# tennisonliu/bayesian-neural-network

Measured on AMD Instinct MI355X. Metric: MC-forward-samples/sec + KL-elements/sec, 784-1200-1200-10 BNN, higher is better.
Workload: dtype bf16

## Files before the change

bayesian-neural-network_amd/csrc/bbb_linear.hip:

```cpp
#include "bnn_device.h"
#include "bnn_fin.h"
#include "bbb_sample_body.h"
#include "bbb_block_gemm.h"
#include "../../include/bnn_hip.h"
#include <string.h>

namespace bnn {

struct BbbK {
  const void* x;
  long x_sstride;
  const float* w_mu;
  const float* w_rho;
  const float* w_sigma;
  const float* b_mu;
  const float* b_rho;
  const float* eps_w;
  const float* eps_b;
  float* eps_w_dump;
  float* eps_b_dump;
  void* y;
  float4* ws;
  int S, B, K, N;
  __bf16* y16;
// ... 801 lines not shown
}

template <int MATH, int R, bool ALIGNED>
__global__ __launch_bounds__(768) void bbb_input_grad_kernel(const BbbK p) {
  bbb_fwd_body<MATH, BNN_F32, R, ALIGNED, false, true>(p, nullptr);
}

template <int NW, bool SIG, int EPS>
__device__ __forceinline__ void bbb_gemm_body(const BbbK& p, float4 (*xt)[8 * 64], float (*bias_s)[16]) {
  const int lane = threadIdx.x & 63, wave = __builtin_amdgcn_readfirstlane(threadIdx.x >> 6);
  const int r = lane & 15, q = lane >> 4;
  const int K = p.K, N = p.N, B = p.B;
  const int tbs = (N + 16 * NW - 1) / (16 * NW), mbs = (B + 127) >> 7;
  const int KS = p.ksl;
  int tb, unit, ks;
  if (!xcd2d_work_item(p.xc, tb, unit, ks)) return;
  const int s = unit / mbs, mb = unit - s * mbs;
  const int item = tb * (p.S * mbs) + unit;
  const int tile = tb * NW + wave;
  const int n = tile * 16 + r;
  const bool n_ok = n < N;
  const int nc = min(n, N - 1);
  const int m0 = mb * 128;
  const int ksteps = (K + 31) >> 5;
  const int spb = (ksteps + KS - 1) / KS, t_lo = ks * spb, t_hi = min(ksteps, t_lo + spb);
  const uint32_t gs = global_sample(p, s);
  const bool do_stats = p.want_stats && mb == 0;
  const bool do_ls = do_stats && s == 0;
  const bool do_dump = mb == 0;
  const int gpr = (K + 3) >> 2;
  const uint32_t wid = p.layer_id * 4u;
  const __bf16* xs = reinterpret_cast<const __bf16*>(p.x) + (size_t)(s / p.xg) * (size_t)p.x_sstride;
  const int T = (N + 15) >> 4;

  if (do_stats && item == 0 && ks == 0 && threadIdx.x == 0) p.ws[0] = make_float4(__int_as_float(T * KS), 0.f, 0.f, 0.f);

  size_t xrow[8 / NW];
#pragma unroll
  for (int i = 0; i < 8 / NW; ++i) xrow[i] = (size_t)min(m0 + (wave + i * NW) * 16 + r, B - 1) * K;
  const uint32_t voff_w = ((uint32_t)nc * (uint32_t)K + (uint32_t)(q * 8)) * 4u, voff_w_max = ((uint32_t)nc * (uint32_t)K + (uint32_t)(K - 8)) * 4u;
  uint32_t voff_x[8 / NW], voff_x_max[8 / NW];
#pragma unroll
  for (int i = 0; i < 8 / NW; ++i) {
    voff_x[i] = ((uint32_t)xrow[i] + (uint32_t)(q * 8)) * 2u;
    voff_x_max[i] = ((uint32_t)xrow[i] + (uint32_t)(K - 8)) * 2u;
  }
  auto stage_dma = [&](int t, int buf) __attribute__((always_inline)) {
#pragma unroll
    for (int i = 0; i < 8 / NW; ++i) {
      const uint32_t vo = min(voff_x[i] + (uint32_t)t * 64u, voff_x_max[i]);
      const uint32_t m0v = (uint32_t)(size_t)(__attribute__((address_space(3))) void*)&xt[buf][(wave + i * NW) * 64];
      asm volatile("s_mov_b32 m0, %2\n\ts_nop 0\n\tglobal_load_lds_dwordx4 %0, %1" ::"v"(vo), "s"(xs), "s"(m0v) : "memory", "m0");
    }
  };

  struct PSet { float4 m_lo, m_hi, g_lo, g_hi; };
  auto load_params = [&](int t, PSet& P) __attribute__((always_inline)) {
    const uint32_t woff = min(voff_w + (uint32_t)t * 128u, voff_w_max);
    const float4* pm = reinterpret_cast<const float4*>(reinterpret_cast<const char*>(p.w_mu) + woff);
    const float4* pg = reinterpret_cast<const float4*>(reinterpret_cast<const char*>(SIG ? p.w_sigma : p.w_rho) + woff);
    P.m_lo = pm[0]; P.m_hi = pm[1]; P.g_lo = pg[0]; P.g_hi = pg[1];
  };

  float bmu_pre = 0.f, brho_pre = 0.f, beps_pre = 0.f;
  if (q == 0 && n_ok && ks == 0) {
    bmu_pre = p.b_mu[n];
    brho_pre = p.b_rho[n];
    beps_pre = bias_eps(p, n, s, gs, do_dump);
  }

  PSet PA, PB;
  PA.m_lo = PA.m_hi = PA.g_lo = PA.g_hi = PB.m_lo = PB.m_hi = PB.g_lo = PB.g_hi = make_float4(0.f, 0.f, 0.f, 0.f);
  if (t_lo < t_hi) {
    load_params(t_lo, PA);
    stage_dma(t_lo, t_lo & 1);
  }
  asm volatile("s_waitcnt vmcnt(0)" ::: "memory");
  __syncthreads();

  f32x4 acc[8];
#pragma unroll
  for (int m = 0; m < 8; ++m) acc[m] = f32x4{0.f, 0.f, 0.f, 0.f};
  float s_e2 = 0.f, s_a = 0.f, s_ls = 0.f;

  auto step = [&](int t, const PSet& P, PSet& Pn, auto more_) __attribute__((always_inline)) {
    constexpr bool more = decltype(more_)::value;
    const int k = t * 32 + q * 8;
    const bool lane_ok = n_ok && k < K;
#ifdef BNN_TUNE
    if (more) {
      if (!(p.tune & 8)) stage_dma(t + 1, (t + 1) & 1);
      if (!(p.tune & 4)) load_params(t + 1, Pn);
    }
#else
    if (more) {
      stage_dma(t + 1, (t + 1) & 1);
      load_params(t + 1, Pn);
    }
#endif
    const float mu[8] = {P.m_lo.x, P.m_lo.y, P.m_lo.z, P.m_lo.w, P.m_hi.x, P.m_hi.y, P.m_hi.z, P.m_hi.w};
    float sg[8] = {P.g_lo.x, P.g_lo.y, P.g_lo.z, P.g_lo.w, P.g_hi.x, P.g_hi.y, P.g_hi.z, P.g_hi.w};
    float e[8], w[8];
    if (EPS == BNN_EPS_PHILOX) {
      const uint32_t g = (uint32_t)n * (uint32_t)gpr + (uint32_t)(k >> 2);
      philox_normal8(g, gs, wid, p.k0, p.k1, e);
    } else if (EPS == BNN_EPS_MEMORY) {
      load8<true>(p.eps_w + ((size_t)s * N + n) * K + k, lane_ok ? 8 : 0, e);
    } else {
#pragma unroll
      for (int j = 0; j < 8; ++j) e[j] = 0.f;
    }
    if (p.eps_w_dump && do_dump) store8<true>(p.eps_w_dump + ((size_t)s * N + n) * K + k, lane_ok ? 8 : 0, e);
    float e2 = 0.f, a = 0.f, ls = 0.f;
#pragma unroll
    for (int j = 0; j < 8; ++j) {
      if (!SIG) sg[j] = softplus(sg[j]);
      w[j] = __builtin_fmaf(sg[j], e[j], mu[j]);
      e2 = __builtin_fmaf(e[j], e[j], e2);
    }
    if (do_stats) {
      if (p.prior_kind == BNN_PRIOR_GAUSS) {
#pragma unroll
        for (int j = 0; j < 8; ++j) a = __builtin_fmaf(w[j], w[j], a);
      } else {
#pragma unroll
        for (int j = 0; j < 8; ++j) a = add_log(a, mix_p(p, w[j]));
      }
      if (do_ls) {
#pragma unroll
        for (int j = 0; j < 8; ++j) ls = add_log(ls, sg[j]);
      }
      s_e2 += lane_ok ? e2 : 0.f;
      s_a += lane_ok ? a : 0.f;
      s_ls += lane_ok ? ls : 0.f;
    }
    bf16x8 wa;
#pragma unroll
    for (int j = 0; j < 8; ++j) wa[j] = lane_ok ? (__bf16)w[j] : (__bf16)0.f;
    const uint32_t xa = (uint32_t)(size_t)(__attribute__((address_space(3))) void*)&xt[t & 1][q * 16 + r];
#ifdef BNN_TUNE
    const bool tune_nolds = (p.tune & 16) != 0, tune_nomfma = (p.tune & 32) != 0;
#else
    constexpr bool tune_nolds = false, tune_nomfma = false;
#endif
#pragma unroll
    for (int h = 0; h < 2; ++h) {
      f32x4 x0, x1, x2, x3;
      if (tune_nolds) {
        x0 = x1 = x2 = x3 = f32x4{mu[0], mu[1], mu[2], mu[3]};
      } else {
        if (h == 0)
          asm volatile("ds_read_b128 %0, %4\n\tds_read_b128 %1, %4 offset:1024\n\tds_read_b128 %2, %4 offset:2048\n\tds_read_b128 %3, %4 offset:3072"
                       : "=&v"(x0), "=&v"(x1), "=&v"(x2), "=&v"(x3) : "v"(xa));
        else
          asm volatile("ds_read_b128 %0, %4 offset:4096\n\tds_read_b128 %1, %4 offset:5120\n\tds_read_b128 %2, %4 offset:6144\n\tds_read_b128 %3, %4 offset:7168"
                       : "=&v"(x0), "=&v"(x1), "=&v"(x2), "=&v"(x3) : "v"(xa));
        asm volatile("s_waitcnt lgkmcnt(0)" : "+v"(x0), "+v"(x1), "+v"(x2), "+v"(x3));
      }
      if (!tune_nomfma) {
        acc[h * 4 + 0] = __builtin_amdgcn_mfma_f32_16x16x32_bf16(wa, __builtin_bit_cast(bf16x8, x0), acc[h * 4 + 0], 0, 0, 0);
        acc[h * 4 + 1] = __builtin_amdgcn_mfma_f32_16x16x32_bf16(wa, __builtin_bit_cast(bf16x8, x1), acc[h * 4 + 1], 0, 0, 0);
        acc[h * 4 + 2] = __builtin_amdgcn_mfma_f32_16x16x32_bf16(wa, __builtin_bit_cast(bf16x8, x2), acc[h * 4 + 2], 0, 0, 0);
        acc[h * 4 + 3] = __builtin_amdgcn_mfma_f32_16x16x32_bf16(wa, __builtin_bit_cast(bf16x8, x3), acc[h * 4 + 3], 0, 0, 0);
      } else {
        asm volatile("" :: "v"(x0), "v"(x1), "v"(x2), "v"(x3));
      }
    }
#ifdef BNN_TUNE
    if (!(p.tune & 2)) asm volatile("s_waitcnt vmcnt(0)" ::: "memory");
    if (!(p.tune & 1)) __syncthreads();
#else
    asm volatile("s_waitcnt vmcnt(0)" ::: "memory");
    __syncthreads();
#endif
  };
  {
    int t = t_lo;
#pragma nounroll
    for (; t + 2 < t_hi; t += 2) {
      step(t, PA, PB, std::true_type{});
      step(t + 1, PB, PA, std::true_type{});
    }
    if (t + 1 < t_hi) {
      step(t, PA, PB, std::true_type{});
      step(t + 1, PB, PA, std::false_type{});
    } else if (t < t_hi) {
      step(t, PA, PB, std::false_type{});
    }
  }

  if (q == 0) {
    float b = 0.f;
    if (n_ok && ks == 0) b = sample_bias(p, bmu_pre, brho_pre, beps_pre, do_stats, do_ls, s_e2, s_a, s_ls);
    bias_s[wave][r] = b;
  }
  if (do_stats) {
    const float a = wave_sum(s_e2), b = wave_sum(s_a), cc = wave_sum(s_ls);
    if (lane == 0 && tile < T) p.ws[1 + ((size_t)s * T + tile) * KS + ks] = make_float4(a, b, cc, 0.f);
  }
  __syncthreads();
  const int nb = tile * 16 + q * 4;
  const bool vec_ok = (N & 3) == 0;
  float bq[4];
#pragma unroll
  for (int i = 0; i < 4; ++i) bq[i] = bias_s[wave][q * 4 + i];
  if (KS > 1) {
    __shared__ uint32_t last_s;
    float4* const unit_part = p.ks_part + (size_t)item * KS * (NW * 8 * 64);
    float4* const mine = unit_part + ((size_t)ks * NW + wave) * (8 * 64) + lane;
#pragma unroll
    for (int m = 0; m < 8; ++m) {
      f32x4 v = acc[m];
#pragma unroll
      for (int i = 0; i < 4; ++i) v[i] += bq[i];
      acc[m] = v;
      asm volatile("global_store_dwordx4 %0, %1, off sc1" ::"v"(mine + m * 64), "v"(v) : "memory");
    }
    asm volatile("s_waitcnt vmcnt(0)" ::: "memory");
    __syncthreads();
    if (threadIdx.x == 0) {
      const uint32_t tk = __hip_atomic_fetch_add(p.ks_ticket + item, 1u, __ATOMIC_RELAXED, __HIP_MEMORY_SCOPE_AGENT);
      last_s = (tk == (uint32_t)KS - 1u) ? 1u : 0u;
    }
    __syncthreads();
    if (last_s == 0u) return;
    if (threadIdx.x == 0) __hip_atomic_store(p.ks_ticket + item, 0u, __ATOMIC_RELAXED, __HIP_MEMORY_SCOPE_AGENT);
    f32x4 sum[8];
#pragma unroll
    for (int m = 0; m < 8; ++m) sum[m] = f32x4{0.f, 0.f, 0.f, 0.f};
#pragma nounroll
    for (int j = 0; j < KS; ++j) {
      f32x4 part[8];
      if (j != ks) {
        const float4* src = unit_part + ((size_t)j * NW + wave) * (8 * 64) + lane;
#pragma unroll
        for (int m = 0; m < 8; ++m)
          asm volatile("global_load_dwordx4 %0, %1, off sc1" : "=v"(part[m]) : "v"(src + m * 64) : "memory");
        asm volatile("s_waitcnt vmcnt(0)" ::: "memory");
      } else {
#pragma unroll
        for (int m = 0; m < 8; ++m) part[m] = acc[m];
      }
#pragma unroll
      for (int m = 0; m < 8; ++m) sum[m] += part[m];
    }
#pragma unroll
    for (int m = 0; m < 8; ++m) acc[m] = sum[m];
#pragma unroll
    for (int i = 0; i < 4; ++i) bq[i] = 0.f;
  }
  if (nb < N) {
#pragma unroll
    for (int m = 0; m < 8; ++m) {
      const int brow = m0 + m * 16 + r;
      if (brow < B) {
        f32x4 v = acc[m];
#pragma unroll
        for (int i = 0; i < 4; ++i) {
          float o = v[i] + bq[i];
          if (p.relu) o = fmaxf(o, 0.f);
          v[i] = o;
        }
        const size_t yoff = ((size_t)s * B + brow) * N + nb;
        if (p.y_bf16) {
          __bf16* yp = reinterpret_cast<__bf16*>(p.y) + yoff;
          if (vec_ok) {
            bf16x4 o;
#pragma unroll
            for (int i = 0; i < 4; ++i) o[i] = (__bf16)v[i];
            *reinterpret_cast<bf16x4*>(yp) = o;
          } else {
#pragma unroll
            for (int i = 0; i < 4; ++i)
              if (nb + i < N) yp[i] = (__bf16)v[i];
          }
        } else {
          float* yp = reinterpret_cast<float*>(p.y) + yoff;
          if (vec_ok) {
            *reinterpret_cast<float4*>(yp) = make_float4(v[0], v[1], v[2], v[3]);
          } else {
#pragma unroll
            for (int i = 0; i < 4; ++i)
              if (nb + i < N) yp[i] = v[i];
          }
        }
      }
    }
  }
}

template <int NW, bool SIG, int EPS>
__global__ __launch_bounds__(NW * 64, 4) void bbb_fwd_gemm_kernel(const BbbK p) {
  __shared__ __attribute__((aligned(16))) float4 xt[2][8 * 64];
  __shared__ float bias_s[NW][16];
  bbb_gemm_body<NW, SIG, EPS>(p, xt, bias_s);
}

template <int NF, int SB, int EPS, int NB = 2, bool X3 = false, int LAY = 0>
__global__ __launch_bounds__(NF * SB * 64, 4) void bbb_fwd_gemm2_kernel(const BbbK p) {
  constexpr int NW = NF * SB;
  constexpr bool XTL = (LAY & 1) != 0, YTL = (LAY & 2) != 0, WTL = (LAY & 4) != 0;
  static_assert(!X3 || LAY == 0, "piece order: bf16 form only");
  static_assert(NB == 2, "two staging buffers");
  constexpr int WPW = 4 / SB;
  constexpr int XPW = 8 / NF;
  constexpr int XT = X3 ? 1024 : 512;
  static_assert(SB == 1 || SB == 2 || SB == 4, "pairs per block");
  static_assert(NF == 2 || NF == 4 || NF == 8, "feature waves per block");
  constexpr int BUF = NF * 256 + SB * XT;
  auto p_idx = [](int buf) { return X3 ? 0 : buf * BUF; };
  auto x_idx = [](int buf) { return X3 ? NF * 256 + buf * (SB * XT) : buf * BUF + NF * 256; };
  __shared__ __attribute__((aligned(16))) float4 sm_all[X3 ? NF * 256 + 2 * SB * XT : NB * BUF + NW * 4];
  float (*bias_s)[16] = reinterpret_cast<float (*)[16]>(sm_all + (X3 ? 0 : NB * BUF));
  const int lane = threadIdx.x & 63, wave = __builtin_amdgcn_readfirstlane(threadIdx.x >> 6);
  const int fw = wave % NF, sb = wave / NF;
  const int r = lane & 15, q = lane >> 4;
  const int K = p.K, N = p.N, B = p.B;
  const int mbs = (B + 127) >> 7;
  const int U = p.S * mbs;
  int tb, ub, in_;
  if (!xcd2d_work_item(p.xc, tb, ub, in_)) return;
  const int unit_raw = ub * SB + sb;
  const bool active = unit_raw < U;
  const int unit = active ? unit_raw : U - 1;
  const int s = unit / mbs, mb = unit - s * mbs;
  const int tile = tb * NF + fw;
  const int n = tile * 16 + r;
  const bool n_ok = n < N;
  const int nc = min(n, N - 1);
  const int m0 = mb * 128;
  const int ksteps = (K + 31) >> 5;
  const uint32_t gs = global_sample(p, s);
  const bool do_stats = p.want_stats && mb == 0 && active;
  const bool do_ls = do_stats && s == 0;
  const bool do_dump = mb == 0 && active;
  const int gpr = (K + 3) >> 2;
  const uint32_t wid = p.layer_id * 4u;
  const __bf16* xs = reinterpret_cast<const __bf16*>(p.x) + (size_t)(s / p.xg) * (size_t)p.x_sstride;
  const __bf16* xs_lo = X3 ? reinterpret_cast<const __bf16*>(p.x_lo) + (size_t)(s / p.xg) * (size_t)p.x_sstride : nullptr;
  const int T = (N + 15) >> 4;

  if (do_stats && tb == 0 && unit == 0 && fw == 0 && lane == 0) p.ws[0] = make_float4(__int_as_float(T), 0.f, 0.f, 0.f);

  const size_t wrow = (size_t)nc * K;
  size_t xrow[XPW];
#pragma unroll
  for (int i = 0; i < XPW; ++i) xrow[i] = (size_t)min(m0 + (fw + i * NF) * 16 + r, B - 1) * K;
  const uint32_t voff_w = ((uint32_t)nc * (uint32_t)K + (uint32_t)(q * 8)) * 4u;
  uint32_t voff_x[XPW];
#pragma unroll
  for (int i = 0; i < XPW; ++i) voff_x[i] = ((uint32_t)xrow[i] + (uint32_t)(q * 8)) * 2u;
  const uint32_t lds0 = (uint32_t)(size_t)(__attribute__((address_space(3))) void*)&sm_all[0];
  auto x_slot = [&](int slot) { return x_idx(slot) + sb * XT; };
  const char* xt_unit = reinterpret_cast<const char*>(xs) + (size_t)mb * (size_t)ksteps * 8192;
  const uint32_t voff_xt = (uint32_t)lane * 16u;
  const char* wt_tile = p.w_pieces + (size_t)tile * (size_t)ksteps * 4096;
  auto stage_w_pieces = [&](int t, int pbuf) __attribute__((always_inline)) {
#pragma unroll
    for (int i = 0; i < WPW; ++i) {
      const int j = sb * WPW + i;
      const char* base = wt_tile + (size_t)t * 4096 + j * 1024;
      const uint32_t m0v = lds0 + (uint32_t)((p_idx(pbuf) + (fw * 4 + j) * 64) * 16);
      asm volatile("s_mov_b32 m0, %2\n\ts_nop 0\n\tglobal_load_lds_dwordx4 %0, %1" ::"v"(voff_xt), "s"(base), "s"(m0v) : "memory", "m0");
    }
  };
  auto stage_x_pieces = [&](int t, int xbuf) __attribute__((always_inline)) {
#pragma unroll
    for (int i = 0; i < XPW; ++i) {
      const char* base = xt_unit + (size_t)t * 8192 + (fw + i * NF) * 1024;
      const uint32_t m0v = lds0 + (uint32_t)((x_slot(xbuf) + (fw + i * NF) * 64) * 16);
      asm volatile("s_mov_b32 m0, %2\n\ts_nop 0\n\tglobal_load_lds_dwordx4 %0, %1" ::"v"(voff_xt), "s"(base), "s"(m0v) : "memory", "m0");
    }
  };
  auto stage_fast = [&](int t, int pbuf, int xbuf, auto wp_, auto wx_) __attribute__((always_inline)) {
    if (WTL && decltype(wp_)::value) {
      stage_w_pieces(t, pbuf);
    } else if (decltype(wp_)::value) {
#pragma unroll
      for (int i = 0; i < WPW; ++i) {
        const int j = sb * WPW + i;
        const char* base = reinterpret_cast<const char*>((j & 2) ? p.w_sigma : p.w_mu) + (size_t)t * 128 + (j & 1) * 16;
        const uint32_t m0v = lds0 + (uint32_t)((p_idx(pbuf) + (fw * 4 + j) * 64) * 16);
        asm volatile("s_mov_b32 m0, %2\n\ts_nop 0\n\tglobal_load_lds_dwordx4 %0, %1" ::"v"(voff_w), "s"(base), "s"(m0v) : "memory", "m0");
      }
    }
    if (XTL && decltype(wx_)::value) {
      stage_x_pieces(t, xbuf);
    } else if (decltype(wx_)::value) {
#pragma unroll
      for (int i = 0; i < XPW; ++i) {
        const char* base = reinterpret_cast<const char*>(xs) + (size_t)t * 64;
        const uint32_t m0v = lds0 + (uint32_t)((x_slot(xbuf) + (fw + i * NF) * 64) * 16);
        asm volatile("s_mov_b32 m0, %2\n\ts_nop 0\n\tglobal_load_lds_dwordx4 %0, %1" ::"v"(voff_x[i]), "s"(base), "s"(m0v) : "memory", "m0");
      }
      if (X3) {
#pragma unroll
        for (int i = 0; i < XPW; ++i) {
          const char* base = reinterpret_cast<const char*>(xs_lo) + (size_t)t * 64;
          const uint32_t m0v = lds0 + (uint32_t)((x_idx(xbuf) + sb * XT + 512 + (fw + i * NF) * 64) * 16);
          asm volatile("s_mov_b32 m0, %2\n\ts_nop 0\n\tglobal_load_lds_dwordx4 %0, %1" ::"v"(voff_x[i]), "s"(base), "s"(m0v) : "memory", "m0");
        }
      }
    }
  };
  auto stage_slow = [&](int t, int pbuf, int xbuf, auto wp_, auto wx_) __attribute__((always_inline)) {
    const int kk = min(t * 32 + q * 8, K - 8);
    if (WTL && decltype(wp_)::value) {
      stage_w_pieces(t, pbuf);
    } else if (decltype(wp_)::value) {
#pragma unroll
      for (int i = 0; i < WPW; ++i) {
#ifdef BNN_TUNE
        const int j = ((p.tune & 64) ? (SB - 1 - sb) : sb) * WPW + i;
#else
        const int j = sb * WPW + i;
#endif
        const float* src = ((j & 2) ? p.w_sigma : p.w_mu) + wrow + kk + (j & 1) * 4;
        __builtin_amdgcn_global_load_lds((const __attribute__((address_space(1))) void*)src,
                                         (__attribute__((address_space(3))) void*)&sm_all[p_idx(pbuf) + (fw * 4 + j) * 64], 16, 0, 0);
      }
    }
    if (XTL && decltype(wx_)::value) {
      stage_x_pieces(t, xbuf);
    } else if (decltype(wx_)::value) {
#pragma unroll
      for (int i = 0; i < XPW; ++i) {
        __builtin_amdgcn_global_load_lds((const __attribute__((address_space(1))) void*)(xs + xrow[i] + kk),
                                         (__attribute__((address_space(3))) void*)&sm_all[x_slot(xbuf) + (fw + i * NF) * 64], 16, 0, 0);
      }
      if (X3) {
#pragma unroll
        for (int i = 0; i < XPW; ++i) {
          __builtin_amdgcn_global_load_lds((const __attribute__((address_space(1))) void*)(xs_lo + xrow[i] + kk),
                                           (__attribute__((address_space(3))) void*)&sm_all[x_idx(xbuf) + sb * XT + 512 + (fw + i * NF) * 64], 16, 0, 0);
        }
      }
    }
  };
  auto stage_sel = [&](int t, int pbuf, int xbuf, auto wp_, auto wx_) __attribute__((always_inline)) {
    if ((t + 1) * 32 <= K) stage_fast(t, pbuf, xbuf, wp_, wx_);
    else stage_slow(t, pbuf, xbuf, wp_, wx_);
  };
  auto stage = [&](int t, int buf) __attribute__((always_inline)) { stage_sel(t, buf, buf, std::true_type{}, std::true_type{}); };
  const bool phantom = tile >= T;

  if (phantom) stage_sel(0, 0, 0, std::false_type{}, std::true_type{});
  else stage(0, 0);
  float bmu_pre = 0.f, brho_pre = 0.f, beps_pre = 0.f;
  if (q == 0 && n_ok) {
    bmu_pre = p.b_mu[n];
    brho_pre = p.b_rho[n];
    beps_pre = bias_eps(p, n, s, gs, do_dump);
  }
  asm volatile("s_waitcnt vmcnt(0)" ::: "memory");
  __syncthreads();

  f32x4 acc[8];
#pragma unroll
  for (int m = 0; m < 8; ++m) acc[m] = f32x4{0.f, 0.f, 0.f, 0.f};
  float s_e2 = 0.f, s_a = 0.f, s_ls = 0.f;

  typedef __attribute__((ext_vector_type(2))) float f32x2;
#ifdef BNN_STAMPS
  unsigned long long ph[5] = {0, 0, 0, 0, 0};
#define K2_T(v) const unsigned long long v = __builtin_amdgcn_s_memtime()
#else
#define K2_T(v)
#endif
  auto mfma_phase = [&](const bf16x8& wa, const bf16x8& wl, int xi, const f32x4& m_lo) __attribute__((always_inline)) {
    const uint32_t xa = lds0 + (uint32_t)((xi + q * 16 + r) * 16);
#ifdef BNN_TUNE
    const bool tune_nolds = (p.tune & 16) != 0, tune_nomfma = (p.tune & 32) != 0;
#else
    constexpr bool tune_nolds = false, tune_nomfma = false;
#endif
#pragma unroll
    for (int h = 0; h < 2; ++h) {
      f32x4 x0, x1, x2, x3;
      if (tune_nolds) {
        x0 = x1 = x2 = x3 = m_lo;
      } else if (h == 0)
        asm volatile("ds_read_b128 %0, %4\n\tds_read_b128 %1, %4 offset:1024\n\tds_read_b128 %2, %4 offset:2048\n\tds_read_b128 %3, %4 offset:3072"
                     : "=&v"(x0), "=&v"(x1), "=&v"(x2), "=&v"(x3) : "v"(xa));
      else
        asm volatile("ds_read_b128 %0, %4 offset:4096\n\tds_read_b128 %1, %4 offset:5120\n\tds_read_b128 %2, %4 offset:6144\n\tds_read_b128 %3, %4 offset:7168"
                     : "=&v"(x0), "=&v"(x1), "=&v"(x2), "=&v"(x3) : "v"(xa));
      if (X3) {
        f32x4 l0, l1, l2, l3;
        if (h == 0)
          asm volatile("ds_read_b128 %0, %4 offset:8192\n\tds_read_b128 %1, %4 offset:9216\n\tds_read_b128 %2, %4 offset:10240\n\tds_read_b128 %3, %4 offset:11264"
                       : "=&v"(l0), "=&v"(l1), "=&v"(l2), "=&v"(l3) : "v"(xa));
        else
          asm volatile("ds_read_b128 %0, %4 offset:12288\n\tds_read_b128 %1, %4 offset:13312\n\tds_read_b128 %2, %4 offset:14336\n\tds_read_b128 %3, %4 offset:15360"
                       : "=&v"(l0), "=&v"(l1), "=&v"(l2), "=&v"(l3) : "v"(xa));
        asm volatile("s_waitcnt lgkmcnt(4)" : "+v"(x0), "+v"(x1), "+v"(x2), "+v"(x3));
        acc[h * 4 + 0] = __builtin_amdgcn_mfma_f32_16x16x32_bf16(wa, __builtin_bit_cast(bf16x8, x0), acc[h * 4 + 0], 0, 0, 0);
        acc[h * 4 + 1] = __builtin_amdgcn_mfma_f32_16x16x32_bf16(wa, __builtin_bit_cast(bf16x8, x1), acc[h * 4 + 1], 0, 0, 0);
        acc[h * 4 + 2] = __builtin_amdgcn_mfma_f32_16x16x32_bf16(wa, __builtin_bit_cast(bf16x8, x2), acc[h * 4 + 2], 0, 0, 0);
        acc[h * 4 + 3] = __builtin_amdgcn_mfma_f32_16x16x32_bf16(wa, __builtin_bit_cast(bf16x8, x3), acc[h * 4 + 3], 0, 0, 0);
        acc[h * 4 + 0] = __builtin_amdgcn_mfma_f32_16x16x32_bf16(wl, __builtin_bit_cast(bf16x8, x0), acc[h * 4 + 0], 0, 0, 0);
        acc[h * 4 + 1] = __builtin_amdgcn_mfma_f32_16x16x32_bf16(wl, __builtin_bit_cast(bf16x8, x1), acc[h * 4 + 1], 0, 0, 0);
        acc[h * 4 + 2] = __builtin_amdgcn_mfma_f32_16x16x32_bf16(wl, __builtin_bit_cast(bf16x8, x2), acc[h * 4 + 2], 0, 0, 0);
        acc[h * 4 + 3] = __builtin_amdgcn_mfma_f32_16x16x32_bf16(wl, __builtin_bit_cast(bf16x8, x3), acc[h * 4 + 3], 0, 0, 0);
        asm volatile("s_waitcnt lgkmcnt(0)" : "+v"(l0), "+v"(l1), "+v"(l2), "+v"(l3));
        acc[h * 4 + 0] = __builtin_amdgcn_mfma_f32_16x16x32_bf16(wa, __builtin_bit_cast(bf16x8, l0), acc[h * 4 + 0], 0, 0, 0);
        acc[h * 4 + 1] = __builtin_amdgcn_mfma_f32_16x16x32_bf16(wa, __builtin_bit_cast(bf16x8, l1), acc[h * 4 + 1], 0, 0, 0);
        acc[h * 4 + 2] = __builtin_amdgcn_mfma_f32_16x16x32_bf16(wa, __builtin_bit_cast(bf16x8, l2), acc[h * 4 + 2], 0, 0, 0);
        acc[h * 4 + 3] = __builtin_amdgcn_mfma_f32_16x16x32_bf16(wa, __builtin_bit_cast(bf16x8, l3), acc[h * 4 + 3], 0, 0, 0);
        continue;
      }
      asm volatile("s_waitcnt lgkmcnt(0)" : "+v"(x0), "+v"(x1), "+v"(x2), "+v"(x3));
      if (!tune_nomfma) {
        acc[h * 4 + 0] = __builtin_amdgcn_mfma_f32_16x16x32_bf16(wa, __builtin_bit_cast(bf16x8, x0), acc[h * 4 + 0], 0, 0, 0);
        acc[h * 4 + 1] = __builtin_amdgcn_mfma_f32_16x16x32_bf16(wa, __builtin_bit_cast(bf16x8, x1), acc[h * 4 + 1], 0, 0, 0);
        acc[h * 4 + 2] = __builtin_amdgcn_mfma_f32_16x16x32_bf16(wa, __builtin_bit_cast(bf16x8, x2), acc[h * 4 + 2], 0, 0, 0);
        acc[h * 4 + 3] = __builtin_amdgcn_mfma_f32_16x16x32_bf16(wa, __builtin_bit_cast(bf16x8, x3), acc[h * 4 + 3], 0, 0, 0);
      } else {
        asm volatile("" :: "v"(x0), "v"(x1), "v"(x2), "v"(x3), "v"(wa));
      }
    }
  };
  auto step = [&, &mfma_phase = mfma_phase](int t, int cur, auto full_) __attribute__((always_inline)) {
    constexpr bool FULL = decltype(full_)::value;
    const int k = t * 32 + q * 8;
    const bool lane_ok = FULL || (n_ok && k < K);
    const bool real = FULL || !phantom;
    K2_T(st0);
    const bool staged = t + 1 < ksteps;
#ifdef BNN_TUNE
    if (staged && !(p.tune & 8)) {
#else
    if (staged) {
#endif
      if (X3 || !real) stage_sel(t + 1, 0, cur ^ 1, std::false_type{}, std::true_type{});
      else stage(t + 1, cur ^ 1);
    }
    const uint32_t pa = lds0 + (uint32_t)((p_idx(cur) + fw * 256 + lane) * 16);
    f32x4 m_lo, m_hi, g_lo, g_hi;
    if (X3) {
      asm volatile("ds_read_b128 %0, %4\n\tds_read_b128 %1, %4 offset:1024\n\tds_read_b128 %2, %4 offset:2048\n\tds_read_b128 %3, %4 offset:3072"
                   : "=&v"(m_lo), "=&v"(m_hi), "=&v"(g_lo), "=&v"(g_hi) : "v"(pa));
      asm volatile("s_waitcnt lgkmcnt(0)" : "+v"(m_lo), "+v"(m_hi), "+v"(g_lo), "+v"(g_hi));
      __builtin_amdgcn_s_barrier();
      asm volatile("" ::: "memory");
#ifdef BNN_TUNE
      if (t + 1 < ksteps && real && !(p.tune & 8)) stage_sel(t + 1, 0, 0, std::true_type{}, std::false_type{});
#else
      if (t + 1 < ksteps && real) stage_sel(t + 1, 0, 0, std::true_type{}, std::false_type{});
#endif
    }
    if (real) {
      if (!X3) {
        asm volatile("ds_read_b128 %0, %4\n\tds_read_b128 %1, %4 offset:1024\n\tds_read_b128 %2, %4 offset:2048\n\tds_read_b128 %3, %4 offset:3072"
                     : "=&v"(m_lo), "=&v"(m_hi), "=&v"(g_lo), "=&v"(g_hi) : "v"(pa));
        asm volatile("s_waitcnt lgkmcnt(0)" : "+v"(m_lo), "+v"(m_hi), "+v"(g_lo), "+v"(g_hi));
      }
      K2_T(st1);
      const f32x2 mu2[4] = {{m_lo[0], m_lo[1]}, {m_lo[2], m_lo[3]}, {m_hi[0], m_hi[1]}, {m_hi[2], m_hi[3]}};
      const f32x2 sg2[4] = {{g_lo[0], g_lo[1]}, {g_lo[2], g_lo[3]}, {g_hi[0], g_hi[1]}, {g_hi[2], g_hi[3]}};
      float e[8];
      if (EPS == BNN_EPS_PHILOX) {
        const uint32_t g = (uint32_t)n * (uint32_t)gpr + (uint32_t)(k >> 2);
        uint4 pa_, pb_;
        philox_pair<>(g, gs, wid, p.k0, p.k1, pa_, pb_);
        box_muller8(pa_, pb_, e);
      } else if (EPS == BNN_EPS_MEMORY) {
        load8<true>(p.eps_w + ((size_t)s * N + n) * K + k, lane_ok ? 8 : 0, e);
      } else {
#pragma unroll
        for (int j = 0; j < 8; ++j) e[j] = 0.f;
      }
      if (p.eps_w_dump && do_dump) store8<true>(p.eps_w_dump + ((size_t)s * N + n) * K + k, lane_ok ? 8 : 0, e);
      f32x2 w2[4], e2v = {0.f, 0.f}, av = {0.f, 0.f};
#pragma unroll
      for (int j = 0; j < 4; ++j) {
        const f32x2 ev = {e[2 * j], e[2 * j + 1]};
        w2[j] = __builtin_elementwise_fma(sg2[j], ev, mu2[j]);
        e2v = __builtin_elementwise_fma(ev, ev, e2v);
      }
      if (do_stats) {
        float a, ls = 0.f;
        if (p.prior_kind == BNN_PRIOR_GAUSS) {
#pragma unroll
          for (int j = 0; j < 4; ++j) av = __builtin_elementwise_fma(w2[j], w2[j], av);
          a = av[0] + av[1];
        } else {
          a = 0.f;
#pragma unroll
          for (int j = 0; j < 4; ++j) {
            a = add_log(a, mix_p(p, w2[j][0]));
            a = add_log(a, mix_p(p, w2[j][1]));
          }
        }
        if (do_ls) {
#pragma unroll
          for (int j = 0; j < 4; ++j) {
            ls = add_log(ls, sg2[j][0]);
            ls = add_log(ls, sg2[j][1]);
          }
        }
        const float e2 = e2v[0] + e2v[1];
        s_e2 += lane_ok ? e2 : 0.f;
        s_a += lane_ok ? a : 0.f;
        s_ls += lane_ok ? ls : 0.f;
      }
      bf16x8 wa, wl = {};
      if (X3) {
        typedef __attribute__((ext_vector_type(2))) __bf16 bf16x2;
        uint32_t hw[4], lw[4];
#pragma unroll
        for (int j = 0; j < 4; ++j) {
          const f32x2 wv = lane_ok ? w2[j] : f32x2{0.f, 0.f};
          const uint32_t hb = __builtin_bit_cast(uint32_t, __builtin_convertvector(wv, bf16x2));
          const f32x2 hf = {__uint_as_float(hb << 16), __uint_as_float(hb & 0xffff0000u)};
          hw[j] = hb;
          lw[j] = __builtin_bit_cast(uint32_t, __builtin_convertvector(wv - hf, bf16x2));
        }
        wa = __builtin_bit_cast(bf16x8, make_uint4(hw[0], hw[1], hw[2], hw[3]));
        wl = __builtin_bit_cast(bf16x8, make_uint4(lw[0], lw[1], lw[2], lw[3]));
      } else {
#pragma unroll
        for (int j = 0; j < 4; ++j) {
          wa[2 * j] = lane_ok ? (__bf16)w2[j][0] : (__bf16)0.f;
          wa[2 * j + 1] = lane_ok ? (__bf16)w2[j][1] : (__bf16)0.f;
        }
      }
#ifdef BNN_STAMPS
      asm volatile("" :: "v"(wa));
#endif
      K2_T(st2);
      mfma_phase(wa, wl, x_idx(cur) + sb * XT, m_lo);
#ifdef BNN_STAMPS
      asm volatile("" :: "v"(acc[0]), "v"(acc[7]));
      K2_T(st3);
      ph[0] += st1 - st0; ph[1] += st2 - st1; ph[2] += st3 - st2;
#endif
    }
#ifdef BNN_TUNE
    if (!(p.tune & 2)) asm volatile("s_waitcnt vmcnt(0) lgkmcnt(0)" ::: "memory");
    if (!(p.tune & 1)) __builtin_amdgcn_s_barrier();
#else
    K2_T(st3w);
    asm volatile("s_waitcnt vmcnt(0) lgkmcnt(0)" ::: "memory");
    K2_T(st4);
    __builtin_amdgcn_s_barrier();
#endif
    asm volatile("" ::: "memory");
#ifdef BNN_STAMPS
    K2_T(st5);
    ph[3] += st4 - st3w; ph[4] += st5 - st4;
#endif
  };
  {
    const bool tile_full = (tile + 1) * 16 <= N;
    const int full_steps = tile_full ? (K >> 5) : 0;
    int t = 0, cur = 0;
#pragma nounroll
    for (; t < full_steps; ++t, cur = (cur + 1 == NB ? 0 : cur + 1)) step(t, cur, std::true_type{});
#pragma nounroll
    for (; t < ksteps; ++t, cur = (cur + 1 == NB ? 0 : cur + 1)) step(t, cur, std::false_type{});
  }

#ifdef BNN_STAMPS
  if (p.dbg && lane == 0 && blockIdx.x < 1024) {
    unsigned long long* d = p.dbg + ((size_t)blockIdx.x * NW + wave) * 8;
    d[0] = ph[0]; d[1] = ph[1]; d[2] = ph[2]; d[3] = ph[3]; d[4] = ph[4]; d[5] = (unsigned long long)ksteps;
  }
#endif
#undef K2_T
  float b_own = 0.f;
  if (q == 0) {
    if (n_ok) b_own = sample_bias(p, bmu_pre, brho_pre, beps_pre, do_stats, do_ls, s_e2, s_a, s_ls);
    if (!X3) bias_s[wave][r] = b_own;
  }
  if (do_stats) {
    const float a = wave_sum(s_e2), b = wave_sum(s_a), cc = wave_sum(s_ls);
    if (lane == 0 && tile < T) p.ws[1 + (size_t)s * T + tile] = make_float4(a, b, cc, 0.f);
  }
  float bq[4];
  if (X3) {
#pragma unroll
    for (int i = 0; i < 4; ++i) bq[i] = __shfl(b_own, q * 4 + i, 64);
  } else {
    __syncthreads();
  }
  if (!active) return;
  const int nb = tile * 16 + q * 4;
  const bool vec_ok = (N & 3) == 0;
  if (!X3) {
#pragma unroll
    for (int i = 0; i < 4; ++i) bq[i] = bias_s[wave][q * 4 + i];
  }
  if (nb >= N) return;
  auto store_tiles = [&](auto fast_, auto ybf_, auto relu_) __attribute__((always_inline)) {
    constexpr bool FAST = decltype(fast_)::value;
    const bool ybf = FAST ? decltype(ybf_)::value : p.y_bf16 != 0;
    const bool relu = FAST ? decltype(relu_)::value : p.relu != 0;
    const size_t esz = ybf ? 2 : 4;
    const size_t y0 = YTL ? (((size_t)unit * ((N + 31) >> 5) + (tile >> 1)) * 8192 + ((2 * (tile & 1) + (q >> 1)) * 16 + r) * 16 + (q & 1) * 8)
                          : (((size_t)s * B + m0 + r) * N + nb) * esz;
    const size_t ystep = YTL ? (size_t)1024 : (size_t)16 * N * esz;
    char* yrow = reinterpret_cast<char*>(p.y) + y0;
    char* lrow = X3 ? reinterpret_cast<char*>(p.y_lo) + y0 : nullptr;
#pragma unroll
    for (int m = 0; m < 8; ++m, yrow += ystep, lrow += X3 ? ystep : 0) {
      if (!FAST && m0 + m * 16 + r >= B) continue;
      f32x4 v = acc[m];
#pragma unroll
      for (int i = 0; i < 4; ++i) {
        float o = v[i] + bq[i];
        if (relu) o = fmaxf(o, 0.f);
        v[i] = o;
      }
      if (ybf) {
        __bf16* yp = reinterpret_cast<__bf16*>(yrow);
        bf16x4 o;
#pragma unroll
        for (int i = 0; i < 4; ++i) o[i] = (__bf16)v[i];
        if (FAST || vec_ok) {
          *reinterpret_cast<bf16x4*>(yp) = o;
        } else {
#pragma unroll
          for (int i = 0; i < 4; ++i)
            if (nb + i < N) yp[i] = o[i];
        }
        if (X3) {
          __bf16* lp = reinterpret_cast<__bf16*>(lrow);
          bf16x4 l;
#pragma unroll
          for (int i = 0; i < 4; ++i) l[i] = (__bf16)(v[i] - (float)o[i]);
          if (FAST || vec_ok) {
            *reinterpret_cast<bf16x4*>(lp) = l;
          } else {
#pragma unroll
            for (int i = 0; i < 4; ++i)
              if (nb + i < N) lp[i] = l[i];
          }
        }
      } else {
        float* yp = reinterpret_cast<float*>(yrow);
        if (FAST || vec_ok) {
          *reinterpret_cast<float4*>(yp) = make_float4(v[0], v[1], v[2], v[3]);
        } else {
#pragma unroll
          for (int i = 0; i < 4; ++i)
            if (nb + i < N) yp[i] = v[i];
        }
      }
    }
  };
  constexpr std::true_type yes{};
  constexpr std::false_type no{};
  if (vec_ok && m0 + 128 <= B) {
    if (p.y_bf16) {
      if (p.relu) store_tiles(yes, yes, yes);
      else store_tiles(yes, yes, no);
    } else {
      if (p.relu) store_tiles(yes, no, yes);
      else store_tiles(yes, no, no);
    }
  } else {
    store_tiles(no, no, no);
  }
}

template <bool SIG, int EPS>
__global__ __launch_bounds__(256, 4) void bbb_fwd_gemm_rider_kernel(const BbbK p, const SampleK sk, int n_main) {
  __shared__ __attribute__((aligned(16))) float4 xt[2][8 * 64];
  __shared__ float bias_s[4][16];
  if ((int)blockIdx.x >= n_main) {
    sample_block(sk, (int)blockIdx.x - n_main, &bias_s[0][0]);
    return;
  }
  bbb_gemm_body<4, SIG, EPS>(p, xt, bias_s);
}

__global__ void bbb_layer_scalars_kernel(const float4* __restrict__ ws, int K, int N, bnn_prior prior,
                                         float* __restrict__ log_prior, float* __restrict__ log_q) {
  __shared__ double scratch[16];
  const int s = blockIdx.x;
  const int T = __float_as_int(ws[0].x);
  double e2 = 0, a = 0, ls = 0;
  for (int t = threadIdx.x; t < T; t += blockDim.x) {
    const float4 v = ws[1 + (size_t)s * T + t];
    const float4 v0 = ws[1 + t];
    e2 += v.x;
    a += v.y;
    ls += v0.z;
  }
  e2 = block_sum(e2, scratch);
  a = block_sum(a, scratch);
  ls = block_sum(ls, scratch);
  if (threadIdx.x == 0) {
    const double cnt = (double)N * K + N;
    const double c0 = -0.91893853320467274178;
    if (log_q) log_q[s] = (float)(cnt * c0 - ls - 0.5 * e2);
    if (log_prior) {
      if (prior.kind == BNN_PRIOR_GAUSS)
        log_prior[s] = (float)(cnt * (c0 - log((double)prior.sigma_p)) -
                               a / (2.0 * (double)prior.sigma_p * (double)prior.sigma_p));
      else
        log_prior[s] = (float)a;
    }
  }
}

}

using namespace bnn;

static constexpr int kMaxSlices = 8;
extern "C" size_t bnn_bbb_linear_fwd_workspace_bytes(int32_t n_samples, int32_t out_features) {
  if (n_samples <= 0 || out_features <= 0) return 0;
  return (1 + (size_t)n_samples * (size_t)(((out_features + 15) / 16) * kMaxSlices)) * 4 * sizeof(float);
}

static size_t split_ticket_bytes(long units) { return (((size_t)units * 4 + 255) / 256) * 256; }
extern "C" size_t bnn_bbb_split_scratch_bytes(int32_t n_samples, int32_t batch, int32_t out_features) {
  if (n_samples <= 0 || batch <= 0 || out_features <= 0) return 0;
  const long units = (long)((out_features + 63) / 64) * n_samples * ((batch + 127) / 128);
  return split_ticket_bytes(units) + (size_t)units * kMaxSlices * (4 * 8 * 64 * 16);
}
extern "C" size_t bnn_bbb_split_scratch_zero_bytes(int32_t n_samples, int32_t batch, int32_t out_features) {
  if (n_samples <= 0 || batch <= 0 || out_features <= 0) return 0;
  return split_ticket_bytes((long)((out_features + 63) / 64) * n_samples * ((batch + 127) / 128));
}

static inline bool aligned16(const void* p) { return (reinterpret_cast<uintptr_t>(p) & 15) == 0; }

namespace {
struct BbbPlan {
  int form;
  int R, nw, mt;
  int tiles;
  int ksl;
  int pairs;
  long blocks;
  size_t lds;
};

constexpr size_t kL2WeightBudget = 2560 * 1024;
constexpr int kGemmPairs = 2;
constexpr int kGemmRing = 2;
constexpr int kGemmPairsX3 = 2;
constexpr int kGemmMinBlocks = 450;
constexpr int kSliceMaxBlocks = 2048;
constexpr long kSliceMinWeights = 250000;
constexpr int kBlockGemmMinBatch = 512;
constexpr int kSliceMinSamples = 4;

void tile_plan(int S, int B, int K, int N, bool aligned, int mt, BbbPlan& pl) {
  const int mbs = (B + 16 * mt - 1) / (16 * mt);
  int R = 1;
  if (aligned)
    while (R < 4 && (long)((N + 16 / R - 1) / (16 / R)) * S * mbs < 120) R *= 2;
  const int F = 16 / R;
  const int ssteps = (K + 32 * R - 1) / (32 * R);
  int spw = 1;
  while ((ssteps + spw - 1) / spw > 12) ++spw;
  int nw = (ssteps + spw - 1) / spw;
  if ((long)((N + F - 1) / F) * S * mbs >= 400 && ssteps >= 8) nw = 4;
  else if (ssteps >= 4) nw = (ssteps >= 12 ? 12 : ssteps) & ~3;
  if (nw > ssteps) nw = ssteps;
  pl.form = BNN_FORM_TILE;
  pl.R = R;
  pl.nw = nw < 1 ? 1 : nw;
  pl.mt = mt;
  pl.tiles = (N + F - 1) / F;
  pl.ksl = 1;
  pl.blocks = (long)pl.tiles * S * mbs;
  pl.lds = ((size_t)pl.nw * mt * 64 * 4 + 16 + 3 * pl.nw) * sizeof(float);
}

double slice_cost_us(long gemm_blocks, int ksteps, int ksl) {
  const long blocks = gemm_blocks * ksl;
  const bool short_slices = (ksteps + ksl - 1) / ksl < 8;
  const long per_cu = (blocks <= 1024 || !short_slices) ? (blocks + 255) / 256 : 4 * ((blocks + 1023) / 1024);
  static const double stretch[5] = {0.0, 2.4, 1.4, 1.27, 1.2};
  double us = 0.5 * (double)per_cu * ((ksteps + ksl - 1) / ksl + 1.5) * stretch[per_cu > 4 ? 4 : per_cu] + 3.2;
  if (ksl > 1) {
    const double mb = (double)blocks * 65536.0 / 1.0e6;
    us += 1.8 + mb / 12.0 * (blocks > 1024 ? 1024.0 / (double)blocks : 1.0);
  }
  return us;
}

int kslices(long gemm_blocks, int K, int min_ksl = 1, int forced = 0) {
  const int ksteps = (K + 31) / 32;
  if (forced > 0) return forced > kMaxSlices ? kMaxSlices : (forced > ksteps ? ksteps : forced);
  if (min_ksl * 2 > ksteps) return 1;
  int best = min_ksl;
  double best_cost = 0;
  for (int ksl = min_ksl; ksl <= kMaxSlices && (ksl == 1 || ksl * 2 <= ksteps); ++ksl) {
    if (ksl > min_ksl && gemm_blocks * ksl > kSliceMaxBlocks) break;
    const double cost = slice_cost_us(gemm_blocks, ksteps, ksl);
    if (ksl == min_ksl || cost < best_cost - 1e-9) {
      best_cost = cost;
      best = ksl;
    }
  }
  return best;
}

template <typename KernelT>
hipError_t allow_big_lds(KernelT kernel, size_t lds) {
  if (lds <= 64 * 1024) return hipSuccess;
  return hipFuncSetAttribute(reinterpret_cast<const void*>(kernel), hipFuncAttributeMaxDynamicSharedMemorySize,
                             160 * 1024);
}
}

static int bbb_plan(const bnn_bbb_fwd_args* a, bool al, BbbPlan& pl, bool allow_block = true) {
  const int S = a->n_samples, B = a->batch, K = a->in_features, N = a->out_features;
  const int mbs = (B + 127) / 128;
  if (allow_block && a->w_sampled && a->x_dtype == BNN_BF16 && !a->w_sampled_t_out && !a->y_bf16_copy &&
      (a->form == BNN_FORM_BLOCK256 || (a->form == BNN_FORM_AUTO && B >= kBlockGemmMinBatch)) &&
      (double)(B > N ? B : N) * K * 2.0 < 2147483648.0) {
    pl.form = BNN_FORM_BLOCK256;
    pl.R = 1; pl.nw = 8; pl.mt = 16; pl.tiles = (N + 15) / 16; pl.ksl = 1;
    pl.blocks = (long)S * ((B + 255) / 256) * ((N + 255) / 256);
    pl.lds = kBgLds;
    return BNN_OK;
  }
  if (a->w_sampled) {
    tile_plan(S, B, K, N, true, 8, pl);
    pl.R = 1;
    pl.mt = 2;
    pl.tiles = (N + 15) / 16;
    pl.blocks = (long)pl.tiles * S * ((B + 31) / 32);
    pl.lds = ((size_t)pl.nw * 2 * 64 * 4 + 16 + 3 * pl.nw) * sizeof(float);
    return BNN_OK;
  }
  const long gemm_blocks = (long)((N + 63) / 64) * S * mbs;
  const bool x3 = a->math == BNN_MATH_BF16X3;
  const bool gemm_ok = al && (a->math == BNN_MATH_BF16 || x3) && a->x_dtype == BNN_BF16 && K >= 8 &&
                       (double)N * K * 4.0 < 4294967295.0 && (double)B * K * 2.0 < 4294967295.0 &&
                       (!x3 || (a->w_sigma && !a->rider && (long)S * mbs >= 2 * kGemmPairsX3 && !(reinterpret_cast<uintptr_t>(a->x_lo) & 15) &&
                                (a->y_dtype != BNN_BF16 || !(reinterpret_cast<uintptr_t>(a->y_lo) & 7))));
  const bool slice_ok = gemm_ok && !x3 && a->split_scratch && !(reinterpret_cast<uintptr_t>(a->split_scratch) & 15) &&
                        a->split_scratch_bytes >= bnn_bbb_split_scratch_bytes(S, B, N);
  int forced = 0;
#ifdef BNN_TUNE
  if (const char* v = getenv("BNN_TUNE_KSL")) forced = atoi(v);
#endif
  const int ksl = slice_ok ? kslices(gemm_blocks, K, a->form == BNN_FORM_GEMM_KSLICE ? 2 : 1, forced) : 1;
  int form = a->form;
  if ((form == BNN_FORM_GEMM && !gemm_ok) || (form == BNN_FORM_GEMM_KSLICE && ksl <= 1)) form = BNN_FORM_AUTO;
  if (a->y_bf16_copy) form = BNN_FORM_TILE;
  if (form == BNN_FORM_AUTO) {
    if (ksl > 1 && (long)K * N >= kSliceMinWeights && S >= kSliceMinSamples) form = BNN_FORM_GEMM_KSLICE;
    else if (gemm_ok && gemm_blocks >= kGemmMinBlocks) form = BNN_FORM_GEMM;
    else form = BNN_FORM_TILE;
  }
  if (form == BNN_FORM_TILE) {
    tile_plan(S, B, K, N, al, 8, pl);
    return BNN_OK;
  }
  pl.form = form;
  pl.R = 1; pl.nw = 4; pl.mt = 8; pl.tiles = (N + 15) / 16;
  pl.ksl = form == BNN_FORM_GEMM_KSLICE ? ksl : 1;
  pl.blocks = gemm_blocks * pl.ksl;
  pl.lds = 2 * 8 * 64 * 16 + 4 * 16 * sizeof(float);
  pl.pairs = 1;
// ... 536 lines not shown
```

Before: 489,100.

## Specialize maskless gemm2 k-steps by stats mode and issue x LDS reads early

The full-tile k-loop of the gemm2 kernel is split into compile-time specialized step bodies (plain, stats, stats+log-sigma) for the Philox Gaussian-prior path. These bodies drop runtime branches on dump, prior kind and stats flags, and they stage the next step unconditionally through a fast staging path, with the last full step falling back to the generic loop. The x-operand LDS reads are issued right after the mu/sigma reads with partial lgkmcnt waits, so their latency overlaps the sampling math before the MFMAs. The cost is more code and register pressure from several loop instantiations plus hand-placed waitcnt ordering that could be fragile.

```diff
diff --git a/bayesian-neural-network_amd/csrc/bbb_linear.hip b/bayesian-neural-network_amd/csrc/bbb_linear.hip
--- a/bayesian-neural-network_amd/csrc/bbb_linear.hip
+++ b/bayesian-neural-network_amd/csrc/bbb_linear.hip
@@ -1127,6 +1127,15 @@
   constexpr bool XTL = (LAY & 1) != 0, YTL = (LAY & 2) != 0, WTL = (LAY & 4) != 0;
   static_assert(!X3 || LAY == 0, "piece order: bf16 form only");
   static_assert(NB == 2, "two staging buffers");
+#ifndef BNN_K1B2_STEP_PARTS
+#define BNN_K1B2_STEP_PARTS 3
+#endif
+  constexpr bool STEP_FORMS = !X3 && (BNN_K1B2_STEP_PARTS & 1);
+#ifdef BNN_TUNE
+  constexpr bool X_EARLY = false;
+#else
+  constexpr bool X_EARLY = !X3 && (BNN_K1B2_STEP_PARTS & 2);
+#endif
   constexpr int WPW = 4 / SB;
   constexpr int XPW = 8 / NF;
   constexpr int XT = X3 ? 1024 : 512;
@@ -1345,19 +1354,29 @@
       }
     }
   };
-  auto step = [&, &mfma_phase = mfma_phase](int t, int cur, auto full_) __attribute__((always_inline)) {
+  auto step = [&, &mfma_phase = mfma_phase](int t, int cur, auto full_, auto body_, auto fast_) __attribute__((always_inline)) {
     constexpr bool FULL = decltype(full_)::value;
+    constexpr int BODY = decltype(body_)::value;
+    constexpr bool FAST = decltype(fast_)::value;
+    static_assert(!BODY || (FULL && !X3 && EPS == BNN_EPS_PHILOX), "step bodies: maskless bf16 steps of the on-chip generator");
+    static_assert(!FAST || (FULL && !X3), "unconditional staging: the maskless bf16 loop");
     const int k = t * 32 + q * 8;
     const bool lane_ok = FULL || (n_ok && k < K);
     const bool real = FULL || !phantom;
+    constexpr bool XE = X_EARLY && (BODY != 0 || (!STEP_FORMS && FULL));
+    const bool st_dump = BODY ? false : (p.eps_w_dump && do_dump);
+    const bool st_stats = BODY ? BODY >= 2 : do_stats;
+    const bool st_gauss = BODY ? true : p.prior_kind == BNN_PRIOR_GAUSS;
+    const bool st_ls = BODY ? BODY == 3 : do_ls;
     K2_T(st0);
-    const bool staged = t + 1 < ksteps;
+    const bool staged = FAST || t + 1 < ksteps;
 #ifdef BNN_TUNE
     if (staged && !(p.tune & 8)) {
 #else
     if (staged) {
 #endif
-      if (X3 || !real) stage_sel(t + 1, 0, cur ^ 1, std::false_type{}, std::true_type{});
+      if (FAST) stage_fast(t + 1, cur ^ 1, cur ^ 1, std::true_type{}, std::true_type{});
+      else if (X3 || !real) stage_sel(t + 1, 0, cur ^ 1, std::false_type{}, std::true_type{});
       else stage(t + 1, cur ^ 1);
     }
     const uint32_t pa = lds0 + (uint32_t)((p_idx(cur) + fw * 256 + lane) * 16);
@@ -1375,17 +1394,25 @@
 #endif
     }
     if (real) {
+      uint32_t g = (uint32_t)n * (uint32_t)gpr + (uint32_t)(k >> 2);
+      f32x4 xe0, xe1, xe2, xe3;
+      const uint32_t xa = lds0 + (uint32_t)((x_idx(cur) + sb * XT + q * 16 + r) * 16);
       if (!X3) {
         asm volatile("ds_read_b128 %0, %4\n\tds_read_b128 %1, %4 offset:1024\n\tds_read_b128 %2, %4 offset:2048\n\tds_read_b128 %3, %4 offset:3072"
                      : "=&v"(m_lo), "=&v"(m_hi), "=&v"(g_lo), "=&v"(g_hi) : "v"(pa));
-        asm volatile("s_waitcnt lgkmcnt(0)" : "+v"(m_lo), "+v"(m_hi), "+v"(g_lo), "+v"(g_hi));
+        if (XE) {
+          asm volatile("ds_read_b128 %0, %5\n\tds_read_b128 %1, %5 offset:1024\n\tds_read_b128 %2, %5 offset:2048\n\tds_read_b128 %3, %5 offset:3072"
+                       : "=&v"(xe0), "=&v"(xe1), "=&v"(xe2), "=&v"(xe3), "+v"(g) : "v"(xa));
+          asm volatile("s_waitcnt lgkmcnt(4)" : "+v"(m_lo), "+v"(m_hi), "+v"(g_lo), "+v"(g_hi));
+        } else {
+          asm volatile("s_waitcnt lgkmcnt(0)" : "+v"(m_lo), "+v"(m_hi), "+v"(g_lo), "+v"(g_hi));
+        }
       }
       K2_T(st1);
       const f32x2 mu2[4] = {{m_lo[0], m_lo[1]}, {m_lo[2], m_lo[3]}, {m_hi[0], m_hi[1]}, {m_hi[2], m_hi[3]}};
       const f32x2 sg2[4] = {{g_lo[0], g_lo[1]}, {g_lo[2], g_lo[3]}, {g_hi[0], g_hi[1]}, {g_hi[2], g_hi[3]}};
       float e[8];
       if (EPS == BNN_EPS_PHILOX) {
-        const uint32_t g = (uint32_t)n * (uint32_t)gpr + (uint32_t)(k >> 2);
         uint4 pa_, pb_;
         philox_pair<>(g, gs, wid, p.k0, p.k1, pa_, pb_);
         box_muller8(pa_, pb_, e);
@@ -1395,7 +1422,7 @@
 #pragma unroll
         for (int j = 0; j < 8; ++j) e[j] = 0.f;
       }
-      if (p.eps_w_dump && do_dump) store8<true>(p.eps_w_dump + ((size_t)s * N + n) * K + k, lane_ok ? 8 : 0, e);
+      if (st_dump) store8<true>(p.eps_w_dump + ((size_t)s * N + n) * K + k, lane_ok ? 8 : 0, e);
       f32x2 w2[4], e2v = {0.f, 0.f}, av = {0.f, 0.f};
 #pragma unroll
       for (int j = 0; j < 4; ++j) {
@@ -1403,9 +1430,9 @@
         w2[j] = __builtin_elementwise_fma(sg2[j], ev, mu2[j]);
         e2v = __builtin_elementwise_fma(ev, ev, e2v);
       }
-      if (do_stats) {
+      if (st_stats) {
         float a, ls = 0.f;
-        if (p.prior_kind == BNN_PRIOR_GAUSS) {
+        if (st_gauss) {
 #pragma unroll
           for (int j = 0; j < 4; ++j) av = __builtin_elementwise_fma(w2[j], w2[j], av);
           a = av[0] + av[1];
@@ -1417,7 +1444,7 @@
             a = add_log(a, mix_p(p, w2[j][1]));
           }
         }
-        if (do_ls) {
+        if (st_ls) {
 #pragma unroll
           for (int j = 0; j < 4; ++j) {
             ls = add_log(ls, sg2[j][0]);
@@ -1454,7 +1481,25 @@
       asm volatile("" :: "v"(wa));
 #endif
       K2_T(st2);
-      mfma_phase(wa, wl, x_idx(cur) + sb * XT, m_lo);
+      if (XE) {
+        f32x4 xl0, xl1, xl2, xl3;
+        asm volatile("ds_read_b128 %0, %4 offset:4096\n\tds_read_b128 %1, %4 offset:5120\n\tds_read_b128 %2, %4 offset:6144\n\tds_read_b128 %3, %4 offset:7168"
+                     : "=&v"(xl0), "=&v"(xl1), "=&v"(xl2), "=&v"(xl3) : "v"(xa), "v"(wa));
+        asm volatile("s_waitcnt lgkmcnt(4)" : "+v"(xe0), "+v"(xe1), "+v"(xe2), "+v"(xe3));
+        acc[0] = __builtin_amdgcn_mfma_f32_16x16x32_bf16(wa, __builtin_bit_cast(bf16x8, xe0), acc[0], 0, 0, 0);
+        acc[1] = __builtin_amdgcn_mfma_f32_16x16x32_bf16(wa, __builtin_bit_cast(bf16x8, xe1), acc[1], 0, 0, 0);
+        acc[2] = __builtin_amdgcn_mfma_f32_16x16x32_bf16(wa, __builtin_bit_cast(bf16x8, xe2), acc[2], 0, 0, 0);
+        acc[3] = __builtin_amdgcn_mfma_f32_16x16x32_bf16(wa, __builtin_bit_cast(bf16x8, xe3), acc[3], 0, 0, 0);
+        __builtin_amdgcn_sched_barrier(0);
+        asm volatile("s_waitcnt lgkmcnt(0)" : "+v"(xl0), "+v"(xl1), "+v"(xl2), "+v"(xl3));
+        acc[4] = __builtin_amdgcn_mfma_f32_16x16x32_bf16(wa, __builtin_bit_cast(bf16x8, xl0), acc[4], 0, 0, 0);
+        acc[5] = __builtin_amdgcn_mfma_f32_16x16x32_bf16(wa, __builtin_bit_cast(bf16x8, xl1), acc[5], 0, 0, 0);
+        acc[6] = __builtin_amdgcn_mfma_f32_16x16x32_bf16(wa, __builtin_bit_cast(bf16x8, xl2), acc[6], 0, 0, 0);
+        acc[7] = __builtin_amdgcn_mfma_f32_16x16x32_bf16(wa, __builtin_bit_cast(bf16x8, xl3), acc[7], 0, 0, 0);
+        __builtin_amdgcn_sched_barrier(0);
+      } else {
+        mfma_phase(wa, wl, x_idx(cur) + sb * XT, m_lo);
+      }
 #ifdef BNN_STAMPS
       asm volatile("" :: "v"(acc[0]), "v"(acc[7]));
       K2_T(st3);
@@ -1479,11 +1524,31 @@
   {
     const bool tile_full = (tile + 1) * 16 <= N;
     const int full_steps = tile_full ? (K >> 5) : 0;
+    constexpr std::true_type yes{};
+    constexpr std::false_type no{};
+    constexpr std::integral_constant<int, 0> generic{};
     int t = 0, cur = 0;
+    if constexpr (STEP_FORMS) {
+      const int fast_steps = full_steps - 1;
+      auto run = [&](auto body_) __attribute__((always_inline)) {
 #pragma nounroll
-    for (; t < full_steps; ++t, cur = (cur + 1 == NB ? 0 : cur + 1)) step(t, cur, std::true_type{});
+        for (; t < fast_steps; ++t, cur ^= 1) step(t, cur, yes, body_, yes);
+      };
+      if constexpr (EPS != BNN_EPS_PHILOX) {
+        run(generic);
+      } else {
+        const bool plain = p.prior_kind == BNN_PRIOR_GAUSS && !(p.eps_w_dump && do_dump);
+        if (!plain) run(generic);
+        else if (do_ls) run(std::integral_constant<int, 3>{});
+        else if (do_stats) run(std::integral_constant<int, 2>{});
+        else run(std::integral_constant<int, 1>{});
+      }
+    } else {
 #pragma nounroll
-    for (; t < ksteps; ++t, cur = (cur + 1 == NB ? 0 : cur + 1)) step(t, cur, std::false_type{});
+      for (; t < full_steps; ++t, cur = (cur + 1 == NB ? 0 : cur + 1)) step(t, cur, yes, generic, no);
+    }
+#pragma nounroll
+    for (; t < ksteps; ++t, cur = (cur + 1 == NB ? 0 : cur + 1)) step(t, cur, no, generic, no);
   }
 
 #ifdef BNN_STAMPS
```

Result: faster. 513,600, median of 6 (+5.0%).
